# haidog-yaqub/EzAudio

Measured on NVIDIA H100. Metric: audio-seconds generated per wall-second (EzAudio-XL, 50-step DDIM, 10 s), higher is better.
Workload: dtype bf16

## Files before the change

### ezaudio_b200/csrc/gemm.cuh

```cuda
#pragma once
#include "common.cuh"

namespace ezb {

constexpr int GEMM_BM = 128;
constexpr int GEMM_BK = 64;
#ifdef EZB_GEMM_DEBUG
#define EZB_DBG(...) __VA_ARGS__
#else
#define EZB_DBG(...)
#endif
constexpr int GEMM_SMEM_BUDGET = 227 * 1024 - 2048;
constexpr int gemm_b_box(int bn) { return bn > 256 ? bn / 2 : bn; }

struct GemmShape {
  int M, N;
  int num_k_blocks;
  int num_m_tiles, num_n_tiles;
  int taps, center, dilation, cin_blocks, T, tiles_per_batch;
  int stride, pad;
  unsigned long long* dbg;
  const char* pf;
  unsigned int pf_bytes;
};
// ... 371 lines not shown
    float rstd = 1.f, nmr = 0.f;
    if (fold && lane < nvalid) fold_row_stats(ep.fin, row0 + lane, rstd, nmr);
    wait();
    const int f_begin = c_begin / 2, f_end = c_end / 2;
#pragma unroll 1
    for (int c = f_begin; c < f_end; c += 64) {
      if (n0 + c >= N) break;
      if (ep.split_stride > 0) {
        uint32_t h[32], g[32];
#pragma unroll 1
        for (int q4 = 0; q4 < 2; ++q4) {
          __syncwarp();
          acc_ld<32>(ar, c + q4 * 32, lane, h);
          acc_ld<32>(ar, HALF + c + q4 * 32, lane, g);
          if (lane < nvalid) {
            __nv_bfloat16* o = ep.out_bf16 + (size_t)(row0 + lane) * ep.ld16 + (n0 / 2 + c + q4 * 32);
#pragma unroll
            for (int j = 0; j < 32; j += 2) {
              const float o0 = (__uint_as_float(h[j]) + ep.bias[n0 + c + q4 * 32 + j]) * gelu_erf(__uint_as_float(g[j]) + ep.bias[n0 + HALF + c + q4 * 32 + j]);
              const float o1 = (__uint_as_float(h[j + 1]) + ep.bias[n0 + c + q4 * 32 + j + 1]) * gelu_erf(__uint_as_float(g[j + 1]) + ep.bias[n0 + HALF + c + q4 * 32 + j + 1]);
              store_bf16x2(o + j, ep.split_stride, o0, o1);
            }
          }
        }
        continue;
      }
      uint32_t pk[32];
#pragma unroll
      for (int q4 = 0; q4 < 2; ++q4) {
        uint32_t h[32], g[32];
        __syncwarp();
        acc_ld<32>(ar, c + q4 * 32, lane, h);
        acc_ld<32>(ar, HALF + c + q4 * 32, lane, g);
        if (fold) {
          const float* bh = ep.fin.v + n0 + c + q4 * 32;
          const float* bg = ep.fin.v + n0 + HALF + c + q4 * 32;
          const float* uh = ep.fin.u + n0 + c + q4 * 32;
          const float* ug = ep.fin.u + n0 + HALF + c + q4 * 32;
#pragma unroll
          for (int j = 0; j < 32; j += 2) {
            const float o0 = geglu_fast(fmaf(__uint_as_float(h[j]), rstd, fmaf(nmr, __ldg(uh + j), __ldg(bh + j))),
                                        fmaf(__uint_as_float(g[j]), rstd, fmaf(nmr, __ldg(ug + j), __ldg(bg + j))));
            const float o1 = geglu_fast(fmaf(__uint_as_float(h[j + 1]), rstd, fmaf(nmr, __ldg(uh + j + 1), __ldg(bh + j + 1))),
                                        fmaf(__uint_as_float(g[j + 1]), rstd, fmaf(nmr, __ldg(ug + j + 1), __ldg(bg + j + 1))));
            pk[q4 * 16 + j / 2] = pack_bf16(o0, o1);
          }
        } else {
        const float* bh = ep.bias + n0 + c + q4 * 32;
        const float* bg = ep.bias + n0 + HALF + c + q4 * 32;
#pragma unroll
        for (int j = 0; j < 32; j += 2) {
          const float o0 = geglu_fast(__uint_as_float(h[j]) + __ldg(bh + j), __uint_as_float(g[j]) + __ldg(bg + j));
          const float o1 = geglu_fast(__uint_as_float(h[j + 1]) + __ldg(bh + j + 1), __uint_as_float(g[j + 1]) + __ldg(bg + j + 1));
          pk[q4 * 16 + j / 2] = pack_bf16(o0, o1);
        }
        }
      }
      __syncwarp();
#pragma unroll
      for (int gq = 0; gq < 16; ++gq) stage_put<32>(st, lane, gq, __uint_as_float(pk[2 * gq]), __uint_as_float(pk[2 * gq + 1]));
      __syncwarp();
      const int hl = lane & 15, hw = lane >> 4;
      __nv_bfloat16* obase = ep.out_bf16 + (size_t)row0 * ep.ld16 + (n0 / 2 + c + 4 * hl);
#pragma unroll 4
      for (int rp = 0; rp < 16; ++rp) {
        const int rr = 2 * rp + hw;
        if (rr < nvalid) *reinterpret_cast<float2*>(obase + (size_t)rr * ep.ld16) = stage_get<32>(st, rr, hl);
      }
    }
  }
};

__device__ __forceinline__ void warpgroup_bar_sync(int wg) {
  if (wg == 0) named_bar_sync(2, 128);
  else named_bar_sync(3, 128);
}
struct EpiGegluFrag {
  using Params = EpiGegluParams;
  static constexpr bool FRAG = true;
  static constexpr int EPI_WARPS = 8;
  static constexpr bool WIDE_REGS = false;
  static constexpr int STAGE_FLOATS = 32 * 32;
  static constexpr int HALF = 128;
  static __device__ __forceinline__ void frag(const Params& ep, const CUtensorMap* out, float (&d)[128], uint8_t* tile, int m0, int n0, int wg, int lg,
                                              int lane) {
    const int q = lane & 3;
    const int r0 = 16 * lg + (lane >> 2);
    const float2* bh = reinterpret_cast<const float2*>(ep.bias + n0) + q;
    const float2* bg = reinterpret_cast<const float2*>(ep.bias + n0 + HALF) + q;
#pragma unroll
    for (int i = 0; i < 16; ++i) {
      const float2 b_h = __ldg(bh + 4 * i), b_g = __ldg(bg + 4 * i);
      const uint32_t lo = pack_bf16(geglu_fast(d[4 * i] + b_h.x, d[64 + 4 * i] + b_g.x), geglu_fast(d[4 * i + 1] + b_h.y, d[64 + 4 * i + 1] + b_g.y));
      const uint32_t hi = pack_bf16(geglu_fast(d[4 * i + 2] + b_h.x, d[64 + 4 * i + 2] + b_g.x), geglu_fast(d[4 * i + 3] + b_h.y, d[64 + 4 * i + 3] + b_g.y));
      uint8_t* p = tile + (i >> 3) * 8192 + r0 * 128 + (((i & 7) ^ (r0 & 7)) << 4) + 4 * q;
      *reinterpret_cast<uint32_t*>(p) = lo;
      *reinterpret_cast<uint32_t*>(p + 8 * 128) = hi;
    }
    fence_proxy_async_smem();
    warpgroup_bar_sync(wg);
    if ((threadIdx.x & 127) == 0) {
      tma_store_2d(out, tile, n0 / 2, m0 + 64 * wg);
      tma_store_2d(out, tile + 8192, n0 / 2 + 64, m0 + 64 * wg);
      bulk_commit_group();
    }
  }
};
template <class E>
constexpr auto epi_frag_impl(int) -> decltype(E::FRAG) { return E::FRAG; }
template <class E>
constexpr bool epi_frag_impl(long) { return false; }
template <class E>
constexpr bool epi_frag() { return epi_frag_impl<E>(0); }

__device__ __forceinline__ int swap_chunk_tokens(int c, int c_end, int t0, int N) {
  int n = c_end - c;
  if (N - t0 < n) n = N - t0;
  return n < 32 ? n : 32;
}
template <int BN>
struct EpiLinearT {
  using Params = EpiLinearParams;
  static constexpr int EPI_WARPS = 8;
  static constexpr bool WIDE_REGS = false;
  static constexpr int STAGE_FLOATS = 0;
  static __device__ __forceinline__ void load_resid(const Params& ep, float (&x)[32], int t0, int nt, int f, bool f_ok) {
#pragma unroll
    for (int j = 0; j < 32; ++j) x[j] = (f_ok && j < nt) ? ep.resid[(size_t)(t0 + j) * ep.ldr + f] : 0.f;
  }
  template <class Wait>
  static __device__ __forceinline__ void run(const Params& ep, float* st, const AccRows& ar, int row0, int nvalid, int n0, int N, int lane, int c_begin,
                                             int c_end, Wait wait) {
    const int f = row0 + lane;
    const bool f_ok = lane < nvalid;
    const float bias = (ep.bias != nullptr && f_ok) ? ep.bias[f] : 0.f;
    bool waited = false;
    float x[32];
    if (ep.resid != nullptr && n0 + c_begin < N) load_resid(ep, x, n0 + c_begin, swap_chunk_tokens(c_begin, c_end, n0 + c_begin, N), f, f_ok);
#pragma unroll 1
    for (int c = c_begin; c < c_end; c += 32) {
      const int t0 = n0 + c;
      if (t0 >= N) break;
      const int nt = swap_chunk_tokens(c, c_end, t0, N);
      float xn[32];
      const bool more = ep.resid != nullptr && c + 32 < c_end && t0 + 32 < N;
      if (more) load_resid(ep, xn, t0 + 32, swap_chunk_tokens(c + 32, c_end, t0 + 32, N), f, f_ok);
      float g0 = 1.f, g1 = 1.f;
      int btok = 0x7fffffff;
      if (ep.gate != nullptr && f_ok) {
        const int b0i = t0 / ep.rows_per_batch;
        btok = (b0i + 1) * ep.rows_per_batch;
        g0 = 1.0f - ep.gate[(size_t)b0i * ep.gate_bstride + f];
        if (btok < t0 + nt) g1 = 1.0f - ep.gate[(size_t)(b0i + 1) * ep.gate_bstride + f];
      }
      if (!waited) { wait(); waited = true; }
      uint32_t r[32];
      __syncwarp();
      acc_ld<32>(ar, c, lane, r);
      if (f_ok) {
        float* o = ep.out_f32 + (size_t)t0 * ep.ld32 + f;
#pragma unroll
        for (int j = 0; j < 32; ++j) {
          if (j >= nt) break;
          float v = __uint_as_float(r[j]) + bias;
          if (ep.resid != nullptr) v = fmaf((t0 + j >= btok) ? g1 : g0, v, x[j]);
          o[(size_t)j * ep.ld32] = v;
        }
      }
// ... 239 lines not shown
  constexpr uint16_t MC_MASK = static_cast<uint16_t>((1u << MC) - 1u);
  uint8_t* smem = smem_raw + ((1024u - (smem_u32(smem_raw) & 1023u)) & 1023u);
  uint8_t* sA = smem;
  uint8_t* sB = smem + STAGES * SM::A_BYTES;
  float* sAcc = reinterpret_cast<float*>(smem);
  float* sStage = reinterpret_cast<float*>(smem + SM::RING);
  uint64_t* full = reinterpret_cast<uint64_t*>(smem + SM::RING + SM::STAGE_BYTES);
  uint64_t* empty = full + STAGES;
  uint64_t* acc_free = empty + STAGES;

  const int warp = threadIdx.x >> 5;
  const int lane = threadIdx.x & 31;
  const int num_tiles = g.num_m_tiles * g.num_n_tiles;
  constexpr int PRODUCER = EPI_WARPS;

  if (warp == PRODUCER && lane == 0) {
    tma_prefetch_desc(&tmA);
    tma_prefetch_desc(&tmB);
    for (int i = 0; i < STAGES; ++i) {
      mbar_init(&full[i], 1);
      mbar_init(&empty[i], SM::MMA_WG * MC);
    }
    mbar_init(acc_free, EPI_WARPS * MC);
    fence_mbar_init();
  }
  __syncthreads();
  if (MC > 1) cluster_sync_all();
  pdl_launch();
  if (warp == PRODUCER && g.pf_bytes != 0) {
    if (elect_one()) prefetch_weights_l2(g.pf, g.pf_bytes, blockIdx.x, gridDim.x);
    __syncwarp();
  }
  pdl_wait();
  EZB_DBG(const bool dbg = g.dbg != nullptr && blockIdx.x == 0; const long long t_start = clock64(); long long w0 = 0, w1 = 0, w4 = 0;)

  if (warp >= PRODUCER) {
    if constexpr (SM::PRODUCER_WG) setmaxnreg_dec<SM::REGS_PRODUCER>();
    uint32_t stage = 0, phase = 0, af_phase = 0;
    bool first = true;
    for (int tile = warp == PRODUCER ? (int)blockIdx.x : num_tiles; tile < num_tiles; tile += gridDim.x) {
      const int mt = tile % g.num_m_tiles, nt = tile / g.num_m_tiles;
      const int n0 = nt * BN;
      if (!SM::FRAG && !first) { mbar_wait(acc_free, af_phase); af_phase ^= 1; }
      first = false;
      for (int kb0 = 0; kb0 < g.num_k_blocks; kb0 += KSUB) {
        EZB_DBG(const long long tq = clock64();)
        mbar_wait(&empty[stage], phase ^ 1);
        EZB_DBG(w0 += clock64() - tq;)
        const int nsub = g.num_k_blocks - kb0 < KSUB ? g.num_k_blocks - kb0 : KSUB;
        if (elect_one()) {
          mbar_expect_tx(&full[stage], nsub * (SM::A_SUB + SM::B_SUB));
          for (int sub = 0; sub < nsub; ++sub) {
          const int kb = kb0 + sub;
          uint8_t* dA = sA + stage * SM::A_BYTES + sub * SM::A_SUB;
          uint8_t* dB = sB + stage * SM::B_BYTES + sub * SM::B_SUB;
          if (g.taps == 0) {
            tma_load_2d(dA, &tmA, &full[stage], kb * KB_ELEMS, mt * GEMM_BM);
          } else {
            const int tap = kb / g.cin_blocks, cb = kb - tap * g.cin_blocks;
            const int bidx = mt / g.tiles_per_batch, t0 = (mt - bidx * g.tiles_per_batch) * GEMM_BM;
            if (g.stride > 1) {
              const int off = tap - g.pad;
              const int r = ((off % g.stride) + g.stride) % g.stride, dq = (off - r) / g.stride;
              tma_load_4d(dA, &tmA, &full[stage], cb * GEMM_BK, r, t0 + dq, bidx);
            } else {
              tma_load_3d(dA, &tmA, &full[stage], cb * GEMM_BK, t0 + (tap - g.center) * g.dilation, bidx);
            }
          }
          if (MC == 1) {
            constexpr int BOX = gemm_b_box(BN);
#pragma unroll
            for (int j = 0; j < BN / BOX; ++j) tma_load_2d(dB + j * BOX * 128, &tmB, &full[stage], kb * KB_ELEMS, n0 + j * BOX);
          } else {
            constexpr int SR = McSub<BN>::ROWS;
            for (int j = (int)cluster_ctarank(); j < BN / SR; j += MC)
              tma_load_2d_mc(dB + j * SR * 128, &tmB, &full[stage], kb * KB_ELEMS, n0 + j * SR, MC_MASK);
          }
          }
        }
        __syncwarp();
        if (++stage == STAGES) { stage = 0; phase ^= 1; }
      }
    }
    if constexpr (SM::PRODUCER_WG) setmaxnreg_inc<SM::REGS_LAUNCH>();
  } else {
    if constexpr (SM::PRODUCER_WG) setmaxnreg_inc<SM::REGS_CONSUMER>();
    const int wg = warp >> 2, lg = warp & 3;
    uint32_t stage = 0, phase = 0;
    if constexpr (SM::FRAG) {
      static_assert(!FP8 && !FIRST_PHASE && KSUB == 1, "FRAG: bf16 kernels of one phase (gemm_frag_kernel)");
      uint8_t* tile_buf = reinterpret_cast<uint8_t*>(sStage) + wg * (SM::STAGE_BYTES / 2);
      for (int tile = blockIdx.x; tile < num_tiles; tile += gridDim.x) {
        const int mt = tile % g.num_m_tiles, nt = tile / g.num_m_tiles;
        EZB_DBG(const long long tm = clock64();)
        float d[NSUB][SM::NH][SM::HN / 2];
        gemm_mainloop<BN, Epi, MC, KSUB>(d, wg * NSUB, sA, sB, full, empty, g.num_k_blocks, stage, phase);
        EZB_DBG(const long long ta = clock64(); w0 += ta - tm;)
        if ((threadIdx.x & 127) == 0) bulk_wait_group_read<0>();
        warpgroup_bar_sync(wg);
        EZB_DBG(const long long te = clock64(); w1 += te - ta;)
        Epi::frag(ep, tmC, d[0][0], tile_buf, mt * GEMM_BM, nt * BN, wg, lg, lane);
        EZB_DBG(w4 += clock64() - te;)
      }
      if ((threadIdx.x & 127) == 0) bulk_wait_group<0>();
    } else
    for (int tile = blockIdx.x; tile < num_tiles; tile += gridDim.x) {
      const int mt = tile % g.num_m_tiles, nt = tile / g.num_m_tiles;
      EZB_DBG(const long long tm = clock64();)
      gemm_mma_part<BN, Epi, MC, KSUB, FP8>(wg * NSUB, sA, sB, sAcc, full, empty, g.num_k_blocks, stage, phase, lg, lane, fs, mt * GEMM_BM, g.M, nt * BN);
      EZB_DBG(const long long ta = clock64(); w0 += ta - tm;)
      named_bar_sync(1, 32 * EPI_WARPS);
      EZB_DBG(const long long te = clock64(); w1 += te - ta;)
      int row0, nvalid;
      if (g.taps == 0) {
        row0 = mt * GEMM_BM + lg * 32;
        nvalid = g.M - row0;
      } else {
        const int bidx = mt / g.tiles_per_batch, t0 = (mt - bidx * g.tiles_per_batch) * GEMM_BM + lg * 32;
        row0 = bidx * g.T + t0;
        nvalid = g.T - t0;
      }
      constexpr int CW = BN / (EPI_WARPS / 4);
      const AccRows ar{sAcc + lg * 32 * SM::ACC_PITCH, SM::ACC_PITCH};
      Epi::run(ep, sStage + warp * Epi::STAGE_FLOATS, ar, row0, nvalid, nt * BN, g.N, lane, wg * CW, (wg + 1) * CW, []() {});
      EZB_DBG(w4 += clock64() - te;)
      fence_proxy_async_smem();
      __syncwarp();
      if (lane == 0) {
        if (MC == 1) mbar_arrive(acc_free);
        else for (int r = 0; r < MC; ++r) mbar_arrive_cluster(mapa_u32(smem_u32(acc_free), r));
      }
    }
    if constexpr (SM::PRODUCER_WG) setmaxnreg_dec<SM::REGS_LAUNCH>();
  }
  EZB_DBG(if (dbg && lane == 0) {
    if (warp == PRODUCER) atomicAdd(&g.dbg[2], (unsigned long long)w0);
    if (warp == 0) {
      atomicAdd(&g.dbg[0], (unsigned long long)w0); atomicAdd(&g.dbg[1], (unsigned long long)w1); atomicAdd(&g.dbg[4], (unsigned long long)w4);
      atomicAdd(&g.dbg[5], (unsigned long long)(clock64() - t_start));
    }
  })
  __syncthreads();
  if (MC > 1) cluster_sync_all();
  if (FIRST_PHASE) {
    if (warp == PRODUCER && lane == 0) {
      for (int i = 0; i < STAGES; ++i) { mbar_inval(&full[i]); mbar_inval(&empty[i]); }
      mbar_inval(acc_free);
    }
    __syncthreads();
  }
}
template <int BN, class Epi, int MC = 1, int KSUB = 1>
__global__ void __launch_bounds__((GemmCfg<BN, Epi, KSUB>::THREADS), 1)
gemm_wgmma_kernel(const __grid_constant__ CUtensorMap tmA, const __grid_constant__ CUtensorMap tmB, const GemmShape g,
                  const typename Epi::Params ep) {
  extern __shared__ uint8_t smem_dyn[];
  gemm_body<BN, Epi, MC, false, KSUB>(tmA, tmB, g, ep, smem_dyn);
}
template <int BN, class Epi>
__global__ void __launch_bounds__((GemmCfg<BN, Epi>::THREADS), 1)
gemm_frag_kernel(const __grid_constant__ CUtensorMap tmA, const __grid_constant__ CUtensorMap tmB, const __grid_constant__ CUtensorMap tmC,
                 const GemmShape g, const typename Epi::Params ep) {
  extern __shared__ uint8_t smem_dyn[];
  gemm_body<BN, Epi, 2>(tmA, tmB, g, ep, smem_dyn, Fp8Scales{}, &tmC);
}
template <int BN, class Epi>
__global__ void __launch_bounds__((GemmCfg<BN, Epi>::THREADS), 1)
gemm_fp8_kernel(const __grid_constant__ CUtensorMap tmA, const __grid_constant__ CUtensorMap tmB, const GemmShape g, const typename Epi::Params ep,
                const Fp8Scales fs) {
  extern __shared__ uint8_t smem_dyn[];
  gemm_body<BN, Epi, 2, false, 1, true>(tmA, tmB, g, ep, smem_dyn, fs);
}

}

namespace ezb {
struct EpiHeadsParams {
  int D, H, L;
  int kind[3];
  float nw[2][72];
  float nb[2][72];
  const float2* rope;
  int rope_ld;
  int rope_mufu;
  float inv_freq[36];
  int rope_kinds;
  __nv_bfloat16* out[3];
  int ld_qk, dvp, Lpad;
  int dbg;
  FoldIn fin;
};

template <int DH, int HPT = 2, bool DIRECT = false, bool FOLD = false, bool DBG = false>
struct EpiHeads {
  using Params = EpiHeadsParams;
  static constexpr int BN = HPT == 3 ? (DH == 72 ? 224 : 3 * DH) : 2 * DH;
  static constexpr int EPI_WARPS = 8;
  static constexpr bool WIDE_REGS = HPT == 3;
  static constexpr int STAGE_FLOATS = DIRECT ? 0 : EPI_STAGE_FLOATS;
  template <class Wait>
  static __device__ __forceinline__ void run(const Params& ep, float* st, const AccRows& ar, int row0, int nvalid, int n0, int N, int lane, int c_begin,
                                             int c_end, Wait wait) {
    const int row = row0 + lane;
    const bool row_ok = lane < nvalid;
    constexpr bool fold = FOLD;
    float f_rstd = 1.f, f_nmr = 0.f;
    if (fold && row_ok) fold_row_stats(ep.fin, row, f_rstd, f_nmr);
    wait();
    const int b = row_ok ? row / ep.L : 0, l = row_ok ? row - b * ep.L : 0;
#pragma unroll 1
    for (int hh = threadIdx.x >> 7; hh < HPT; hh += 2) {
      int sec, head;
      if (HPT == 3) {
        const int g = (n0 / BN) * 3 + hh;
        sec = g / ep.H;
        head = g - sec * ep.H;
      } else {
        const int n = n0 + hh * DH;
        if (n >= N) break;
        sec = n / ep.D;
        head = (n - sec * ep.D) / DH;
      }
      const int kind = ep.kind[sec];
      uint32_t r[DH];
      __syncwarp();
      acc_ld<64>(ar, hh * DH, lane, r);
      if constexpr (DH == 72) acc_ld<8>(ar, hh * DH + 64, lane, r + 64);
      float v[DH];
#pragma unroll
      for (int i = 0; i < DH; ++i) v[i] = __uint_as_float(r[i]);
      if (fold) {
        const float4* u4 = reinterpret_cast<const float4*>(ep.fin.u + n0 + hh * DH);
        const float4* v4 = reinterpret_cast<const float4*>(ep.fin.v + n0 + hh * DH);
#pragma unroll
        for (int i = 0; i < DH / 4; ++i) {
          const float4 uu = __ldg(u4 + i), vv = __ldg(v4 + i);
          v[4 * i] = fmaf(v[4 * i], f_rstd, fmaf(f_nmr, uu.x, vv.x));
          v[4 * i + 1] = fmaf(v[4 * i + 1], f_rstd, fmaf(f_nmr, uu.y, vv.y));
          v[4 * i + 2] = fmaf(v[4 * i + 2], f_rstd, fmaf(f_nmr, uu.z, vv.z));
          v[4 * i + 3] = fmaf(v[4 * i + 3], f_rstd, fmaf(f_nmr, uu.w, vv.w));
        }
      }
      const size_t bh = (size_t)b * ep.H + head;
      if (kind < 2) {
        float s1[4] = {0.f, 0.f, 0.f, 0.f}, s2[4] = {0.f, 0.f, 0.f, 0.f};
#pragma unroll
        for (int i = 0; i < DH; ++i) { s1[i & 3] += v[i]; s2[i & 3] = fmaf(v[i], v[i], s2[i & 3]); }
        const float mean = ((s1[0] + s1[1]) + (s1[2] + s1[3])) * (1.0f / DH);
        const float var = fmaxf(((s2[0] + s2[1]) + (s2[2] + s2[3])) * (1.0f / DH) - mean * mean, 0.f);
        const float rstd = rsqrtf(var + 1e-5f);
        const float nmr = -mean * rstd;
        if (DBG && (ep.dbg & 2)) {
        } else if (kind == 0) {
#pragma unroll
          for (int i = 0; i < DH; ++i) v[i] = fmaf(fmaf(v[i], rstd, nmr), ep.nw[0][i], ep.nb[0][i]);
        } else {
#pragma unroll
          for (int i = 0; i < DH; ++i) v[i] = fmaf(fmaf(v[i], rstd, nmr), ep.nw[1][i], ep.nb[1][i]);
        }
        if (ep.rope != nullptr && ((ep.rope_kinds >> kind) & 1) && !(DBG && (ep.dbg & 1))) {
          const float2* cs = ep.rope + (size_t)l * (DH / 2);
          const float lf = (float)l;
#pragma unroll
          for (int i = 0; i < DH / 2; ++i) {
            float2 c;
            if (ep.rope_mufu) __sincosf(lf * ep.inv_freq[i], &c.y, &c.x);
            else c = __ldg(cs + i);
            const float a = v[i], bq = v[i + DH / 2];
            v[i] = a * c.x - bq * c.y;
            v[i + DH / 2] = bq * c.x + a * c.y;
          }
        }
        if constexpr (DIRECT) {
          if (row_ok) {
            uint4* dst = reinterpret_cast<uint4*>(ep.out[kind] + (bh * ep.L + l) * (size_t)ep.ld_qk);
#pragma unroll
            for (int g = 0; g < DH / 8; ++g)
              dst[g] = make_uint4(pack_bf16(v[8 * g], v[8 * g + 1]), pack_bf16(v[8 * g + 2], v[8 * g + 3]), pack_bf16(v[8 * g + 4], v[8 * g + 5]),
                                  pack_bf16(v[8 * g + 6], v[8 * g + 7]));
          }
          continue;
        }
#pragma unroll
        for (int g = 0; g < DH / 4; ++g)
          stage_put(st, lane, g, __uint_as_float(pack_bf16(v[4 * g], v[4 * g + 1])), __uint_as_float(pack_bf16(v[4 * g + 2], v[4 * g + 3])));
        __syncwarp();
        if (lane < DH / 4 && !(DBG && (ep.dbg & 8))) {
          const int rb0 = row0 / ep.L, rl0 = row0 - rb0 * ep.L;
          __nv_bfloat16* base = ep.out[kind] + 4 * lane;
          const size_t head_rows = (size_t)ep.L * ep.ld_qk;
          const int nv = nvalid < 32 ? nvalid : 32;
#pragma unroll 4
          for (int rr = 0; rr < nv; ++rr) {
            int rl = rl0 + rr, rb = rb0;
            while (rl >= ep.L) { rl -= ep.L; ++rb; }
            *reinterpret_cast<float2*>(base + ((size_t)rb * ep.H + head) * head_rows + (size_t)rl * ep.ld_qk) = stage_get(st, rr, lane);
          }
        }
      } else if (row_ok && !(DBG && (ep.dbg & 4))) {
        __nv_bfloat16* dst = ep.out[2] + bh * ep.dvp * ep.Lpad + l;
#pragma unroll
        for (int i = 0; i < DH; ++i) { *dst = __float2bfloat16_rn(v[i]); dst += ep.Lpad; }
        for (int i = DH; i < ep.dvp; ++i) { *dst = __float2bfloat16_rn(0.f); dst += ep.Lpad; }
      }
    }
  }
};

}

namespace ezb {
struct GridBarrier { unsigned int count; unsigned int gen; };
__device__ __forceinline__ void grid_barrier(GridBarrier* b) {
  __syncthreads();
  if (threadIdx.x == 0) {
    __threadfence();
    unsigned int gen;
    asm volatile("ld.acquire.gpu.global.u32 %0, [%1];" : "=r"(gen) : "l"(&b->gen) : "memory");
    if (atomicAdd(&b->count, 1u) == gridDim.x - 1) {
      b->count = 0;
      __threadfence();
      asm volatile("st.release.gpu.global.u32 [%0], %1;" ::"l"(&b->gen), "r"(gen + 1) : "memory");
    } else {
      unsigned int cur;
      do {
        asm volatile("ld.acquire.gpu.global.u32 %0, [%1];" : "=r"(cur) : "l"(&b->gen) : "memory");
      } while (cur == gen);
    }
  }
  __syncthreads();
  asm volatile("fence.proxy.async;" ::: "memory");
}
template <int BN1, class Epi1, class Epi2>
__global__ void __launch_bounds__((GemmCfg<BN1, Epi1>::THREADS), 1)
mlp_fused_kernel(const __grid_constant__ CUtensorMap tmA1, const __grid_constant__ CUtensorMap tmB1, const GemmShape g1, const typename Epi1::Params ep1,
                 const __grid_constant__ CUtensorMap tmA2, const __grid_constant__ CUtensorMap tmB2, const GemmShape g2, const typename Epi2::Params ep2,
                 GridBarrier* bar) {
  static_assert(GemmCfg<BN1, Epi1>::THREADS == GemmCfg<256, Epi2>::THREADS, "both phases use the same warp roles");
  extern __shared__ uint8_t smem_dyn[];
  gemm_body<BN1, Epi1, 2, true>(tmA1, tmB1, g1, ep1, smem_dyn);
  grid_barrier(bar);
  gemm_body<256, Epi2, 1>(tmA2, tmB2, g2, ep2, smem_dyn);
}

}
```

### ezaudio_b200/csrc/host.cuh

```cuda
#pragma once
#include <cuda.h>
#include <cuda_runtime.h>
#include <stdarg.h>
#include <stdio.h>
#include <stdlib.h>
#include <string.h>

#include <map>
#include <string>
#include <tuple>
#include <utility>
#include <vector>

#include "../../include/ezb200.h"
#include "gemm.cuh"

namespace ezb {


inline unsigned long long& launch_counter() {
  static unsigned long long n = 0;
  return n;
}
inline int& opt_pair_gemm() {
// ... 323 lines not shown
  EZB_TRY(dev.tmaps.get2d(A, (uint64_t)K, (uint64_t)M_tokens, (uint64_t)lda, gemm_b_box(BN), &tB));
  return launch_gemm_t<BN, Epi>(dev, st, tA, tB, g, ep);
}

inline int swapped_bn(const Device& dev, int M_tokens, int N_features) {
  const long long mt = (N_features + GEMM_BM - 1) / GEMM_BM;
  auto span = [&](long long bn) { return (mt * ((M_tokens + bn - 1) / bn) + dev.num_sms - 1) / dev.num_sms * bn; };
  return span(288) < span(256) ? 288 : 256;
}
template <template <int> class Epi>
int gemm_swapped(Device& dev, cudaStream_t st, const __nv_bfloat16* A, int lda, const __nv_bfloat16* W, int ldw, int M_tokens, int N_features, int K,
                 const typename Epi<256>::Params& ep) {
  if (swapped_bn(dev, M_tokens, N_features) == 288) return gemm_swapped_at<288, Epi<288>>(dev, st, A, lda, W, ldw, M_tokens, N_features, K, ep);
  return gemm_swapped_at<256, Epi<256>>(dev, st, A, lda, W, ldw, M_tokens, N_features, K, ep);
}

inline int& opt_swap_mc() {
  static int v = 0;
  return v;
}
template <template <int> class EpiT, int MC>
int gemm_swapped_mc(Device& dev, cudaStream_t st, const __nv_bfloat16* A, int lda, const __nv_bfloat16* W, int ldw, int M_tokens, int N_features, int K,
                    const typename EpiT<256>::Params& ep) {
  constexpr int BN = 256;
  using Epi = EpiT<BN>;
  const int mt = (N_features + GEMM_BM - 1) / GEMM_BM, nt = (M_tokens + BN - 1) / BN, tiles = mt * nt;
  auto kern = gemm_wgmma_kernel<BN, Epi, MC>;
  constexpr int smem = GemmCfg<BN, Epi>::BYTES;
  constexpr int GEMM_THREADS = GemmCfg<BN, Epi>::THREADS;
  static int max_clusters[16] = {};
  int& mc = max_clusters[dev.id & 15];
  if (mc == 0) {
    mc = -1;
    if (cudaFuncSetAttribute(kern, cudaFuncAttributeMaxDynamicSharedMemorySize, smem) == cudaSuccess) {
      cudaLaunchConfig_t cfg;
      memset(&cfg, 0, sizeof cfg);
      cfg.gridDim = dim3(MC * 64); cfg.blockDim = dim3(GEMM_THREADS); cfg.dynamicSmemBytes = smem;
      cudaLaunchAttribute at;
      at.id = cudaLaunchAttributeClusterDimension; at.val.clusterDim.x = MC; at.val.clusterDim.y = 1; at.val.clusterDim.z = 1;
      cfg.attrs = &at; cfg.numAttrs = 1;
      int n = 0;
      if (cudaOccupancyMaxActiveClusters(&n, kern, &cfg) == cudaSuccess && n > 0) mc = n;
    }
    (void)cudaGetLastError();
  }
  if (mc <= 0 || (mt % MC) || tiles > mc * MC || (K % 8) || (lda % 8) || (ldw % 8))
    return gemm_swapped<EpiT>(dev, st, A, lda, W, ldw, M_tokens, N_features, K, ep);
  GemmShape g;
  memset(&g, 0, sizeof g);
  g.M = N_features; g.N = M_tokens;
  g.num_m_tiles = mt; g.num_n_tiles = nt;
  g.num_k_blocks = (K + GEMM_BK - 1) / GEMM_BK;
  const CUtensorMap *tA, *tB;
  EZB_TRY(dev.tmaps.get2d(W, (uint64_t)K, (uint64_t)N_features, (uint64_t)ldw, GEMM_BM, &tA));
  EZB_TRY(dev.tmaps.get2d(A, (uint64_t)K, (uint64_t)M_tokens, (uint64_t)lda, 32, &tB));
  GemmProf& gp = gemm_prof();
  cudaEvent_t e0 = nullptr, e1 = nullptr;
  if (gp.on) {
    if (gp.used + 2 > gp.ev.size()) {
      for (int i = 0; i < 2; ++i) { cudaEvent_t e; EZB_CUDA(cudaEventCreate(&e)); gp.ev.push_back(e); }
    }
    e0 = gp.ev[gp.used]; e1 = gp.ev[gp.used + 1];
    gp.used += 2;
    gp.flops.push_back(2.0 * (double)g.M * (double)g.N * (double)g.num_k_blocks * GEMM_BK);
    EZB_CUDA(cudaEventRecord(e0, st));
  }
  EZB_TRY(launch_k(kern, dim3(tiles), dim3(GEMM_THREADS), smem, st, MC, *tA, *tB, g, ep));
  if (gp.on) EZB_CUDA(cudaEventRecord(e1, st));
  return EZB_OK;
}

template <class Kern>
int resident_clusters2(Device& dev, Kern kern, int smem, int threads, int* n) {
  cudaLaunchConfig_t cfg;
  memset(&cfg, 0, sizeof cfg);
  cfg.gridDim = dim3(dev.num_sms & ~1); cfg.blockDim = dim3(threads); cfg.dynamicSmemBytes = smem;
  cudaLaunchAttribute at;
  at.id = cudaLaunchAttributeClusterDimension; at.val.clusterDim.x = 2; at.val.clusterDim.y = 1; at.val.clusterDim.z = 1;
  cfg.attrs = &at; cfg.numAttrs = 1;
  EZB_CUDA(cudaOccupancyMaxActiveClusters(n, kern, &cfg));
  if (*n <= 0) return fail(EZB_ERR_CUDA, "no 2-CTA cluster of this GEMM fits on the device");
  return EZB_OK;
}
template <int BN, class Epi, int KSUB = 1>
int gemm2(Device& dev, cudaStream_t st, const __nv_bfloat16* A, int lda, const __nv_bfloat16* W, int ldw, int M, int N, int K,
          const typename Epi::Params& ep) {
  if (M <= 0 || N <= 0 || K <= 0) return fail(EZB_ERR_SHAPE, "gemm2: empty problem %d %d %d", M, N, K);
  if ((K % 8) || (lda % 8) || (ldw % 8) || (N % 8)) return fail(EZB_ERR_SHAPE, "gemm2: K/ld/N must be multiples of 8 (M%d N%d K%d)", M, N, K);
  GemmShape g;
  memset(&g, 0, sizeof g);
  g.M = M; g.N = N;
  g.num_n_tiles = (N + BN - 1) / BN;
  g.dbg = gemm_dbg_buf();
  g.num_m_tiles = ((M + GEMM_BM - 1) / GEMM_BM + 1) & ~1;
  g.num_k_blocks = (K + GEMM_BK - 1) / GEMM_BK;
  dev.next_weights(W, (size_t)N * ldw * 2, &g.pf, &g.pf_bytes);
  const CUtensorMap *tA, *tB;
  EZB_TRY(dev.tmaps.get2d(A, (uint64_t)K, (uint64_t)M, (uint64_t)lda, GEMM_BM, &tA));
  EZB_TRY(dev.tmaps.get2d(W, (uint64_t)K, (uint64_t)N, (uint64_t)ldw, McSub<BN>::ROWS, &tB));
  constexpr bool FRAG = GemmCfg<BN, Epi, KSUB>::FRAG;
  const CUtensorMap* tC = nullptr;
  if constexpr (FRAG) {
    if (ep.split_stride != 0 || ep.fin.u != nullptr || N % BN)
      return fail(EZB_ERR_ARG, "gemm2: the fragment GEGLU epilogue writes plain bf16 of whole %d-column tiles (N %d)", BN, N);
    EZB_TRY(dev.tmaps.get2d(ep.out_bf16, (uint64_t)N / 2, (uint64_t)M, (uint64_t)ep.ld16, 64, &tC));
  }
  auto kern = [] {
    if constexpr (FRAG) return gemm_frag_kernel<BN, Epi>;
    else return gemm_wgmma_kernel<BN, Epi, 2, KSUB>;
  }();
  constexpr int smem = GemmCfg<BN, Epi, KSUB>::BYTES;
  constexpr int GEMM_THREADS = GemmCfg<BN, Epi, KSUB>::THREADS;
  static int clusters[16] = {};
  if (!clusters[dev.id & 15]) {
    EZB_CUDA(cudaFuncSetAttribute(kern, cudaFuncAttributeMaxDynamicSharedMemorySize, smem));
    EZB_TRY(resident_clusters2(dev, kern, smem, GEMM_THREADS, &clusters[dev.id & 15]));
  }
  const int tiles = g.num_m_tiles * g.num_n_tiles, max_ctas = 2 * clusters[dev.id & 15];
  const int ctas = tiles < max_ctas ? tiles : max_ctas;
  GemmProf& gp = gemm_prof();
  cudaEvent_t e0 = nullptr, e1 = nullptr;
  if (gp.on) {
    if (gp.used + 2 > gp.ev.size()) {
      for (int i = 0; i < 2; ++i) { cudaEvent_t e; EZB_CUDA(cudaEventCreate(&e)); gp.ev.push_back(e); }
    }
    e0 = gp.ev[gp.used]; e1 = gp.ev[gp.used + 1];
    gp.used += 2;
    gp.flops.push_back(2.0 * (double)M * (double)N * (double)g.num_k_blocks * GEMM_BK);
    EZB_CUDA(cudaEventRecord(e0, st));
  }
  if constexpr (FRAG) EZB_TRY(launch_k(kern, dim3(ctas), dim3(GEMM_THREADS), smem, st, 2, *tA, *tB, *tC, g, ep));
  else EZB_TRY(launch_k(kern, dim3(ctas), dim3(GEMM_THREADS), smem, st, 2, *tA, *tB, g, ep));
  if (gp.on) EZB_CUDA(cudaEventRecord(e1, st));
  return EZB_OK;
}

inline int gemm2_geglu(Device& dev, cudaStream_t st, const __nv_bfloat16* A, int lda, const __nv_bfloat16* W, int ldw, int M, int N, int K,
                       const EpiGegluParams& p) {
  const bool tma_out = (reinterpret_cast<uintptr_t>(p.out_bf16) & 15) == 0 && p.ld16 % 8 == 0;
  if (p.split_stride == 0 && N % 256 == 0 && tma_out) return gemm2<256, EpiGegluFrag>(dev, st, A, lda, W, ldw, M, N, K, p);
  return gemm2<256, EpiGeglu<256>>(dev, st, A, lda, W, ldw, M, N, K, p);
}

template <int BN, class Epi>
int gemm2_fp8(Device& dev, cudaStream_t st, const uint8_t* A, const float* sa, const uint8_t* W, const float* sw, int M, int N, int K,
              const typename Epi::Params& ep) {
  if (M <= 0 || N <= 0 || K <= 0) return fail(EZB_ERR_SHAPE, "gemm2_fp8: empty problem %d %d %d", M, N, K);
  if ((K % 16) || (N % BN)) return fail(EZB_ERR_SHAPE, "gemm2_fp8: K must be a multiple of 16 and N of %d (M%d N%d K%d)", BN, M, N, K);
  GemmShape g;
  memset(&g, 0, sizeof g);
  g.M = M; g.N = N;
  g.num_n_tiles = N / BN;
  g.num_m_tiles = ((M + GEMM_BM - 1) / GEMM_BM + 1) & ~1;
  g.num_k_blocks = (K + 2 * GEMM_BK - 1) / (2 * GEMM_BK);
  dev.next_weights(W, (size_t)N * K, &g.pf, &g.pf_bytes);
  const CUtensorMap *tA, *tB;
  EZB_TRY(dev.tmaps.get2d_u8(A, (uint64_t)K, (uint64_t)M, (uint64_t)K, GEMM_BM, &tA));
  EZB_TRY(dev.tmaps.get2d_u8(W, (uint64_t)K, (uint64_t)N, (uint64_t)K, McSub<BN>::ROWS, &tB));
  auto kern = gemm_fp8_kernel<BN, Epi>;
  constexpr int smem = GemmCfg<BN, Epi>::BYTES;
  constexpr int GEMM_THREADS = GemmCfg<BN, Epi>::THREADS;
  static int clusters[16] = {};
  if (!clusters[dev.id & 15]) {
    EZB_CUDA(cudaFuncSetAttribute(kern, cudaFuncAttributeMaxDynamicSharedMemorySize, smem));
    EZB_TRY(resident_clusters2(dev, kern, smem, GEMM_THREADS, &clusters[dev.id & 15]));
  }
  const int tiles = g.num_m_tiles * g.num_n_tiles, max_ctas = 2 * clusters[dev.id & 15];
  const int ctas = tiles < max_ctas ? tiles : max_ctas;
  GemmProf& gp = gemm_prof();
  cudaEvent_t e0 = nullptr, e1 = nullptr;
  if (gp.on) {
    if (gp.used + 2 > gp.ev.size()) {
      for (int i = 0; i < 2; ++i) { cudaEvent_t e; EZB_CUDA(cudaEventCreate(&e)); gp.ev.push_back(e); }
    }
    e0 = gp.ev[gp.used]; e1 = gp.ev[gp.used + 1];
    gp.used += 2;
    gp.flops.push_back(2.0 * (double)M * (double)N * (double)K);
    EZB_CUDA(cudaEventRecord(e0, st));
  }
  const Fp8Scales fs{sa, sw};
  EZB_TRY(launch_k(kern, dim3(ctas), dim3(GEMM_THREADS), smem, st, 2, *tA, *tB, g, ep, fs));
  if (gp.on) EZB_CUDA(cudaEventRecord(e1, st));
  return EZB_OK;
}

inline int& opt_mlp_fused() {
  static int v = [] { const char* e = getenv("EZB_MLP_FUSED"); return e ? atoi(e) : 0; }();
  return v;
}
template <class Epi1, class Epi2>
int mlp_fused(Device& dev, cudaStream_t st, const __nv_bfloat16* A1, const __nv_bfloat16* W1, int M, int N1, int K1, const typename Epi1::Params& ep1,
              const __nv_bfloat16* mid, const __nv_bfloat16* W2, int N2, int K2, const typename Epi2::Params& ep2, GridBarrier* bar) {
  constexpr int BN1 = 256, BN2 = 256;
  if ((K1 % 8) || (K2 % 8) || (N1 % 8)) return fail(EZB_ERR_SHAPE, "mlp_fused: K / N must be multiples of 8");
  GemmShape g1, g2;
  memset(&g1, 0, sizeof g1);
  memset(&g2, 0, sizeof g2);
  g1.M = M; g1.N = N1;
  g1.num_n_tiles = (N1 + BN1 - 1) / BN1; g1.num_m_tiles = ((M + GEMM_BM - 1) / GEMM_BM + 1) & ~1; g1.num_k_blocks = (K1 + GEMM_BK - 1) / GEMM_BK;
  g2.M = N2; g2.N = M;
  g2.num_m_tiles = (N2 + GEMM_BM - 1) / GEMM_BM; g2.num_n_tiles = (M + BN2 - 1) / BN2; g2.num_k_blocks = (K2 + GEMM_BK - 1) / GEMM_BK;
  const CUtensorMap *tA1, *tB1, *tA2, *tB2;
  EZB_TRY(dev.tmaps.get2d(A1, (uint64_t)K1, (uint64_t)M, (uint64_t)K1, GEMM_BM, &tA1));
  EZB_TRY(dev.tmaps.get2d(W1, (uint64_t)K1, (uint64_t)N1, (uint64_t)K1, McSub<BN1>::ROWS, &tB1));
  EZB_TRY(dev.tmaps.get2d(W2, (uint64_t)K2, (uint64_t)N2, (uint64_t)K2, GEMM_BM, &tA2));
  EZB_TRY(dev.tmaps.get2d(mid, (uint64_t)K2, (uint64_t)M, (uint64_t)K2, BN2, &tB2));
  auto kern = mlp_fused_kernel<BN1, Epi1, Epi2>;
  constexpr int s1 = GemmCfg<BN1, Epi1>::BYTES, s2 = GemmCfg<BN2, Epi2>::BYTES, smem = s1 > s2 ? s1 : s2;
  constexpr int THREADS = GemmCfg<BN1, Epi1>::THREADS;
  static int clusters[16] = {};
  if (!clusters[dev.id & 15]) {
    EZB_CUDA(cudaFuncSetAttribute(kern, cudaFuncAttributeMaxDynamicSharedMemorySize, smem));
    EZB_TRY(resident_clusters2(dev, kern, smem, THREADS, &clusters[dev.id & 15]));
  }
  const int grid = 2 * clusters[dev.id & 15];
  return launch_k(kern, dim3(grid), dim3(THREADS), smem, st, 2, *tA1, *tB1, g1, ep1, *tA2, *tB2, g2, ep2, bar);
}

template <int BN, class Epi>
int gemm(Device& dev, cudaStream_t st, const __nv_bfloat16* A, int lda, const __nv_bfloat16* W, int ldw, int M, int N, int K,
         const typename Epi::Params& ep, const ConvAddr* conv = nullptr) {
  if (M <= 0 || N <= 0 || K <= 0) return fail(EZB_ERR_SHAPE, "gemm: empty problem %d %d %d", M, N, K);
  if ((K % 8) || (lda % 8) || (ldw % 8) || (N % 8)) return fail(EZB_ERR_SHAPE, "gemm: K/ld/N must be multiples of 8 (M%d N%d K%d)", M, N, K);
  GemmShape g;
  memset(&g, 0, sizeof g);
  g.M = M;
  g.N = N;
  g.num_n_tiles = (N + BN - 1) / BN;
  dev.next_weights(W, (size_t)N * ldw * 2, &g.pf, &g.pf_bytes);
  const CUtensorMap *tA, *tB;
  if (conv && conv->taps > 0) {
    g.taps = conv->taps;
    g.center = conv->center;
    g.dilation = conv->dilation;
    g.cin_blocks = conv->cin_pad / GEMM_BK;
    g.T = conv->T;
    g.tiles_per_batch = (conv->T + GEMM_BM - 1) / GEMM_BM;
    g.num_m_tiles = g.tiles_per_batch * conv->B;
    g.num_k_blocks = conv->taps * g.cin_blocks;
    g.stride = conv->stride;
    g.pad = conv->pad;
    if (conv->stride > 1) {
      TmapCache::Key k(A, (uint64_t)K, (uint64_t)conv->T, (uint64_t)conv->B, (uint64_t)lda * 1000003ull + conv->stride, GEMM_BM, 4);
      auto it = dev.tmaps.maps.find(k);
      if (it == dev.tmaps.maps.end()) {
        CUtensorMap m;
        EZB_TRY(make_tmap4_strided(&m, A, (uint64_t)K, (uint64_t)conv->stride, (uint64_t)conv->T, (uint64_t)conv->B, (uint64_t)lda));
        it = dev.tmaps.maps.emplace(k, m).first;
      }
      tA = &it->second;
    } else
    EZB_TRY(dev.tmaps.get3d(A, (uint64_t)K, (uint64_t)conv->T, (uint64_t)conv->B, (uint64_t)lda, (uint64_t)lda * conv->T, GEMM_BM, &tA));
    EZB_TRY(dev.tmaps.get2d(W, (uint64_t)conv->taps * conv->cin_pad, (uint64_t)N, (uint64_t)ldw, BN, &tB));
  } else {
    g.num_m_tiles = (M + GEMM_BM - 1) / GEMM_BM;
    g.num_k_blocks = (K + GEMM_BK - 1) / GEMM_BK;
    EZB_TRY(dev.tmaps.get2d(A, (uint64_t)K, (uint64_t)M, (uint64_t)lda, GEMM_BM, &tA));
    EZB_TRY(dev.tmaps.get2d(W, (uint64_t)K, (uint64_t)N, (uint64_t)ldw, BN, &tB));
  }
  return launch_gemm_t<BN, Epi>(dev, st, tA, tB, g, ep);
}

enum HeadsVariant {
  HEADS_PACKED3 = 0,
  HEADS_PACKED3_DIRECT = 1,
  HEADS_PACKED3_KSUB2 = 2,
  HEADS_PAIR = 3,
  HEADS_PAIR_DIRECT = 4,
  HEADS_SINGLE = 5,
};
inline int heads_gemm(Device& dev, cudaStream_t st, const __nv_bfloat16* A, const __nv_bfloat16* W, int M, int N, int dh, int variant,
                      const EpiHeadsParams& e) {
  const int D = e.D, H = e.H;
  const bool fo = e.fin.u != nullptr;
  const bool packed = variant == HEADS_PACKED3 || variant == HEADS_PACKED3_DIRECT || variant == HEADS_PACKED3_KSUB2;
  const bool direct = variant == HEADS_PACKED3_DIRECT || variant == HEADS_PAIR_DIRECT;
  if (dh != 72 && dh != 64) return fail(EZB_ERR_UNSUPPORTED, "heads_gemm: head dimension %d", dh);
  if (packed && N != 3 * D) return fail(EZB_ERR_SHAPE, "heads_gemm: the packed-3 layout holds q, k and v (N %d, D %d)", N, D);
#define EZB_HEADS(BN_, DH_, HPT_, N_)                                                                                                          \
  (fo ? (direct ? gemm2<BN_, EpiHeads<DH_, HPT_, true, true>>(dev, st, A, D, W, D, M, N_, D, e) : gemm2<BN_, EpiHeads<DH_, HPT_, false, true>>(dev, st, A, D, W, D, M, N_, D, e)) \
      : (direct ? gemm2<BN_, EpiHeads<DH_, HPT_, true, false>>(dev, st, A, D, W, D, M, N_, D, e) : gemm2<BN_, EpiHeads<DH_, HPT_, false, false>>(dev, st, A, D, W, D, M, N_, D, e)))
  if (e.dbg) {
    if (variant != HEADS_PACKED3 || dh != 72 || fo) return fail(EZB_ERR_UNSUPPORTED, "heads_gemm: the profiling epilogue is packed-3, dh 72, unfolded");
    return gemm2<224, EpiHeads<72, 3, false, false, true>>(dev, st, A, D, W, D, M, H * 224, D, e);
  }
  switch (variant) {
    case HEADS_PACKED3_KSUB2:
      if (dh != 72 || fo) return fail(EZB_ERR_UNSUPPORTED, "heads_gemm: 128-deep slots exist for dh 72 without fold only");
      return gemm2<224, EpiHeads<72, 3, true, false>, 2>(dev, st, A, D, W, D, M, H * 224, D, e);
    case HEADS_PACKED3:
    case HEADS_PACKED3_DIRECT:
      if (dh == 72) return EZB_HEADS(224, 72, 3, H * 224);
      return EZB_HEADS(192, 64, 3, H * 192);
    case HEADS_PAIR:
    case HEADS_PAIR_DIRECT:
      if (dh == 72) return EZB_HEADS(144, 72, 2, N);
      return EZB_HEADS(128, 64, 2, N);
    case HEADS_SINGLE:
      if (fo) return fail(EZB_ERR_UNSUPPORTED, "heads_gemm: the single-CTA heads kernel has no fold");
      if (dh == 72) return gemm<144, EpiHeads<72>>(dev, st, A, D, W, D, M, N, D, e);
      return gemm<128, EpiHeads<64>>(dev, st, A, D, W, D, M, N, D, e);
  }
#undef EZB_HEADS
  return fail(EZB_ERR_ARG, "heads_gemm: variant %d", variant);
}
inline int heads_gemm_fp8(Device& dev, cudaStream_t st, const uint8_t* A, const float* sa, const uint8_t* W, const float* sw, int M, int dh,
                          const EpiHeadsParams& e) {
  if (e.fin.u != nullptr || e.dbg) return fail(EZB_ERR_UNSUPPORTED, "heads_gemm_fp8: no fold or profiling epilogue");
  if (dh == 72) return gemm2_fp8<224, EpiHeads<72, 3>>(dev, st, A, sa, W, sw, M, e.H * 224, e.D, e);
  if (dh == 64) return gemm2_fp8<192, EpiHeads<64, 3>>(dev, st, A, sa, W, sw, M, e.H * 192, e.D, e);
  return fail(EZB_ERR_UNSUPPORTED, "heads_gemm_fp8: head dimension %d", dh);
}

}
```

Baseline: 49.22.

## Add register-fragment epilogue for QKV heads GEMM with per-head LN and RoPE

Adds an EpiHeadsFrag epilogue that keeps the wgmma accumulators in registers and stages one head slice at a time through a small padded shared-memory buffer. Each thread then applies LayerNorm and RoPE to its row and stores it directly. This replaces the generic accumulator-staging path for the packed-3 and pair heads variants when there is no fold and outputs are 16-byte aligned. It also factors the per-head math into shared helpers and moves the producer's register re-raise to after the final syncthreads. The new path adds extra warpgroup barriers per head and zero-initializes the accumulators, which may raise register pressure.

```diff
diff --git a/ezaudio_b200/csrc/gemm.cuh b/ezaudio_b200/csrc/gemm.cuh
--- a/ezaudio_b200/csrc/gemm.cuh
+++ b/ezaudio_b200/csrc/gemm.cuh
@@ -477,8 +477,8 @@
   static constexpr bool WIDE_REGS = false;
   static constexpr int STAGE_FLOATS = 32 * 32;
   static constexpr int HALF = 128;
-  static __device__ __forceinline__ void frag(const Params& ep, const CUtensorMap* out, float (&d)[128], uint8_t* tile, int m0, int n0, int wg, int lg,
-                                              int lane) {
+  static __device__ __forceinline__ void frag(const Params& ep, const CUtensorMap* out, float (&d)[128], uint8_t* tile, int m0, int n0, const GemmShape&,
+                                              int wg, int lg, int lane) {
     const int q = lane & 3;
     const int r0 = 16 * lg + (lane >> 2);
     const float2* bh = reinterpret_cast<const float2*>(ep.bias + n0) + q;
@@ -884,7 +884,6 @@
         if (++stage == STAGES) { stage = 0; phase ^= 1; }
       }
     }
-    if constexpr (SM::PRODUCER_WG) setmaxnreg_inc<SM::REGS_LAUNCH>();
   } else {
     if constexpr (SM::PRODUCER_WG) setmaxnreg_inc<SM::REGS_CONSUMER>();
     const int wg = warp >> 2, lg = warp & 3;
@@ -895,13 +894,13 @@
       for (int tile = blockIdx.x; tile < num_tiles; tile += gridDim.x) {
         const int mt = tile % g.num_m_tiles, nt = tile / g.num_m_tiles;
         EZB_DBG(const long long tm = clock64();)
-        float d[NSUB][SM::NH][SM::HN / 2];
+        float d[NSUB][SM::NH][SM::HN / 2] = {};
         gemm_mainloop<BN, Epi, MC, KSUB>(d, wg * NSUB, sA, sB, full, empty, g.num_k_blocks, stage, phase);
         EZB_DBG(const long long ta = clock64(); w0 += ta - tm;)
         if ((threadIdx.x & 127) == 0) bulk_wait_group_read<0>();
         warpgroup_bar_sync(wg);
         EZB_DBG(const long long te = clock64(); w1 += te - ta;)
-        Epi::frag(ep, tmC, d[0][0], tile_buf, mt * GEMM_BM, nt * BN, wg, lg, lane);
+        Epi::frag(ep, tmC, d[0][0], tile_buf, mt * GEMM_BM, nt * BN, g, wg, lg, lane);
         EZB_DBG(w4 += clock64() - te;)
       }
       if ((threadIdx.x & 127) == 0) bulk_wait_group<0>();
@@ -943,6 +942,7 @@
     }
   })
   __syncthreads();
+  if constexpr (SM::PRODUCER_WG) if (warp >= PRODUCER) setmaxnreg_inc<SM::REGS_LAUNCH>();
   if (MC > 1) cluster_sync_all();
   if (FIRST_PHASE) {
     if (warp == PRODUCER && lane == 0) {
@@ -993,10 +993,72 @@
   FoldIn fin;
 };
 
+constexpr int heads_bn(int dh, int hpt) { return hpt == 3 ? (dh == 72 ? 224 : 3 * dh) : 2 * dh; }
+template <int DH, int HPT>
+__device__ __forceinline__ bool head_of_tile(const EpiHeadsParams& ep, int n0, int hh, int N, int& sec, int& head) {
+  if (HPT == 3) {
+    const int g = (n0 / heads_bn(DH, HPT)) * 3 + hh;
+    sec = g / ep.H;
+    head = g - sec * ep.H;
+    return true;
+  }
+  const int n = n0 + hh * DH;
+  if (n >= N) return false;
+  sec = n / ep.D;
+  head = (n - sec * ep.D) / DH;
+  return true;
+}
+template <int DH, bool DBG>
+__device__ __forceinline__ void head_ln_rope(const EpiHeadsParams& ep, float (&v)[DH], int kind, int l) {
+  float s1[4] = {0.f, 0.f, 0.f, 0.f}, s2[4] = {0.f, 0.f, 0.f, 0.f};
+#pragma unroll
+  for (int i = 0; i < DH; ++i) { s1[i & 3] += v[i]; s2[i & 3] = fmaf(v[i], v[i], s2[i & 3]); }
+  const float mean = ((s1[0] + s1[1]) + (s1[2] + s1[3])) * (1.0f / DH);
+  const float var = fmaxf(((s2[0] + s2[1]) + (s2[2] + s2[3])) * (1.0f / DH) - mean * mean, 0.f);
+  const float rstd = rsqrtf(var + 1e-5f);
+  const float nmr = -mean * rstd;
+  if (DBG && (ep.dbg & 2)) {
+  } else if (kind == 0) {
+#pragma unroll
+    for (int i = 0; i < DH; ++i) v[i] = fmaf(fmaf(v[i], rstd, nmr), ep.nw[0][i], ep.nb[0][i]);
+  } else {
+#pragma unroll
+    for (int i = 0; i < DH; ++i) v[i] = fmaf(fmaf(v[i], rstd, nmr), ep.nw[1][i], ep.nb[1][i]);
+  }
+  if (ep.rope != nullptr && ((ep.rope_kinds >> kind) & 1) && !(DBG && (ep.dbg & 1))) {
+    const float2* cs = ep.rope + (size_t)l * (DH / 2);
+    const float lf = (float)l;
+#pragma unroll
+    for (int i = 0; i < DH / 2; ++i) {
+      float2 c;
+      if (ep.rope_mufu) __sincosf(lf * ep.inv_freq[i], &c.y, &c.x);
+      else c = __ldg(cs + i);
+      const float a = v[i], bq = v[i + DH / 2];
+      v[i] = a * c.x - bq * c.y;
+      v[i + DH / 2] = bq * c.x + a * c.y;
+    }
+  }
+}
+template <int DH>
+__device__ __forceinline__ void head_store_row(const EpiHeadsParams& ep, const float (&v)[DH], int kind, size_t bh, int l) {
+  uint4* dst = reinterpret_cast<uint4*>(ep.out[kind] + (bh * ep.L + l) * (size_t)ep.ld_qk);
+#pragma unroll
+  for (int g = 0; g < DH / 8; ++g)
+    dst[g] = make_uint4(pack_bf16(v[8 * g], v[8 * g + 1]), pack_bf16(v[8 * g + 2], v[8 * g + 3]), pack_bf16(v[8 * g + 4], v[8 * g + 5]),
+                        pack_bf16(v[8 * g + 6], v[8 * g + 7]));
+}
+template <int DH>
+__device__ __forceinline__ void head_store_vt(const EpiHeadsParams& ep, const float (&v)[DH], size_t bh, int l) {
+  __nv_bfloat16* dst = ep.out[2] + bh * ep.dvp * ep.Lpad + l;
+#pragma unroll
+  for (int i = 0; i < DH; ++i) { *dst = __float2bfloat16_rn(v[i]); dst += ep.Lpad; }
+  for (int i = DH; i < ep.dvp; ++i) { *dst = __float2bfloat16_rn(0.f); dst += ep.Lpad; }
+}
+
 template <int DH, int HPT = 2, bool DIRECT = false, bool FOLD = false, bool DBG = false>
 struct EpiHeads {
   using Params = EpiHeadsParams;
-  static constexpr int BN = HPT == 3 ? (DH == 72 ? 224 : 3 * DH) : 2 * DH;
+  static constexpr int BN = heads_bn(DH, HPT);
   static constexpr int EPI_WARPS = 8;
   static constexpr bool WIDE_REGS = HPT == 3;
   static constexpr int STAGE_FLOATS = DIRECT ? 0 : EPI_STAGE_FLOATS;
@@ -1013,16 +1075,7 @@
 #pragma unroll 1
     for (int hh = threadIdx.x >> 7; hh < HPT; hh += 2) {
       int sec, head;
-      if (HPT == 3) {
-        const int g = (n0 / BN) * 3 + hh;
-        sec = g / ep.H;
-        head = g - sec * ep.H;
-      } else {
-        const int n = n0 + hh * DH;
-        if (n >= N) break;
-        sec = n / ep.D;
-        head = (n - sec * ep.D) / DH;
-      }
+      if (!head_of_tile<DH, HPT>(ep, n0, hh, N, sec, head)) break;
       const int kind = ep.kind[sec];
       uint32_t r[DH];
       __syncwarp();
@@ -1045,42 +1098,9 @@
       }
       const size_t bh = (size_t)b * ep.H + head;
       if (kind < 2) {
-        float s1[4] = {0.f, 0.f, 0.f, 0.f}, s2[4] = {0.f, 0.f, 0.f, 0.f};
-#pragma unroll
-        for (int i = 0; i < DH; ++i) { s1[i & 3] += v[i]; s2[i & 3] = fmaf(v[i], v[i], s2[i & 3]); }
-        const float mean = ((s1[0] + s1[1]) + (s1[2] + s1[3])) * (1.0f / DH);
-        const float var = fmaxf(((s2[0] + s2[1]) + (s2[2] + s2[3])) * (1.0f / DH) - mean * mean, 0.f);
-        const float rstd = rsqrtf(var + 1e-5f);
-        const float nmr = -mean * rstd;
-        if (DBG && (ep.dbg & 2)) {
-        } else if (kind == 0) {
-#pragma unroll
-          for (int i = 0; i < DH; ++i) v[i] = fmaf(fmaf(v[i], rstd, nmr), ep.nw[0][i], ep.nb[0][i]);
-        } else {
-#pragma unroll
-          for (int i = 0; i < DH; ++i) v[i] = fmaf(fmaf(v[i], rstd, nmr), ep.nw[1][i], ep.nb[1][i]);
-        }
-        if (ep.rope != nullptr && ((ep.rope_kinds >> kind) & 1) && !(DBG && (ep.dbg & 1))) {
-          const float2* cs = ep.rope + (size_t)l * (DH / 2);
-          const float lf = (float)l;
-#pragma unroll
-          for (int i = 0; i < DH / 2; ++i) {
-            float2 c;
-            if (ep.rope_mufu) __sincosf(lf * ep.inv_freq[i], &c.y, &c.x);
-            else c = __ldg(cs + i);
-            const float a = v[i], bq = v[i + DH / 2];
-            v[i] = a * c.x - bq * c.y;
-            v[i + DH / 2] = bq * c.x + a * c.y;
-          }
-        }
+        head_ln_rope<DH, DBG>(ep, v, kind, l);
         if constexpr (DIRECT) {
-          if (row_ok) {
-            uint4* dst = reinterpret_cast<uint4*>(ep.out[kind] + (bh * ep.L + l) * (size_t)ep.ld_qk);
-#pragma unroll
-            for (int g = 0; g < DH / 8; ++g)
-              dst[g] = make_uint4(pack_bf16(v[8 * g], v[8 * g + 1]), pack_bf16(v[8 * g + 2], v[8 * g + 3]), pack_bf16(v[8 * g + 4], v[8 * g + 5]),
-                                  pack_bf16(v[8 * g + 6], v[8 * g + 7]));
-          }
+          if (row_ok) head_store_row<DH>(ep, v, kind, bh, l);
           continue;
         }
 #pragma unroll
@@ -1100,10 +1120,64 @@
           }
         }
       } else if (row_ok && !(DBG && (ep.dbg & 4))) {
-        __nv_bfloat16* dst = ep.out[2] + bh * ep.dvp * ep.Lpad + l;
-#pragma unroll
-        for (int i = 0; i < DH; ++i) { *dst = __float2bfloat16_rn(v[i]); dst += ep.Lpad; }
-        for (int i = DH; i < ep.dvp; ++i) { *dst = __float2bfloat16_rn(0.f); dst += ep.Lpad; }
+        head_store_vt<DH>(ep, v, bh, l);
+      }
+    }
+  }
+};
+
+template <int DH, int HPT>
+struct EpiHeadsFrag {
+  using Params = EpiHeadsParams;
+  static constexpr bool FRAG = true;
+  static constexpr int BN = heads_bn(DH, HPT);
+  static constexpr int EPI_WARPS = 8;
+  static constexpr bool WIDE_REGS = true;
+  static constexpr int PITCH = DH + 4;
+  static constexpr int STAGE_FLOATS = 64 * PITCH / 4;
+  static_assert(DH % 8 == 0, "head slices start on a fragment register quad");
+  static __device__ __forceinline__ void frag(const Params& ep, const CUtensorMap*, float (&d)[BN / 2], uint8_t* tile, int m0, int n0, const GemmShape& g,
+                                              int wg, int lg, int lane) {
+    float* buf = reinterpret_cast<float*>(tile);
+    const int t = threadIdx.x & 127, half = t >> 6;
+    const int row = m0 + 64 * wg + (t & 63);
+    const bool row_ok = row < g.M;
+    const int b = row_ok ? row / ep.L : 0, l = row_ok ? row - b * ep.L : 0;
+    float* w0 = buf + (16 * lg + (lane >> 2)) * PITCH + 2 * (lane & 3);
+    const float4* rd = reinterpret_cast<const float4*>(buf + (t & 63) * PITCH);
+#pragma unroll
+    for (int p = 0; p < HPT; p += 2) {
+      float v[DH];
+#pragma unroll
+      for (int s = 0; s < 2; ++s) {
+        const int hh = p + s;
+        if (hh >= HPT) break;
+        if (hh > 0) warpgroup_bar_sync(wg);
+#pragma unroll
+        for (int i = 0; i < DH / 8; ++i) {
+          const int j = 4 * (hh * DH / 8 + i);
+          *reinterpret_cast<float2*>(w0 + 8 * i) = make_float2(d[j], d[j + 1]);
+          *reinterpret_cast<float2*>(w0 + 8 * PITCH + 8 * i) = make_float2(d[j + 2], d[j + 3]);
+        }
+        warpgroup_bar_sync(wg);
+        if (half == s) {
+#pragma unroll
+          for (int i = 0; i < DH / 4; ++i) {
+            const float4 x = rd[i];
+            v[4 * i] = x.x; v[4 * i + 1] = x.y; v[4 * i + 2] = x.z; v[4 * i + 3] = x.w;
+          }
+        }
+      }
+      const int hh = p + half;
+      int sec, head;
+      if (hh >= HPT || !head_of_tile<DH, HPT>(ep, n0, hh, g.N, sec, head)) continue;
+      const int kind = ep.kind[sec];
+      const size_t bh = (size_t)b * ep.H + head;
+      if (kind < 2) {
+        head_ln_rope<DH, false>(ep, v, kind, l);
+        if (row_ok) head_store_row<DH>(ep, v, kind, bh, l);
+      } else if (row_ok) {
+        head_store_vt<DH>(ep, v, bh, l);
       }
     }
   }
diff --git a/ezaudio_b200/csrc/host.cuh b/ezaudio_b200/csrc/host.cuh
--- a/ezaudio_b200/csrc/host.cuh
+++ b/ezaudio_b200/csrc/host.cuh
@@ -429,6 +429,17 @@
   if (*n <= 0) return fail(EZB_ERR_CUDA, "no 2-CTA cluster of this GEMM fits on the device");
   return EZB_OK;
 }
+inline int frag_out_map(Device& dev, const EpiGegluParams& ep, int M, int N, int BN, const CUtensorMap** tC) {
+  if (ep.split_stride != 0 || ep.fin.u != nullptr || N % BN)
+    return fail(EZB_ERR_ARG, "gemm2: the fragment GEGLU epilogue writes plain bf16 of whole %d-column tiles (N %d)", BN, N);
+  return dev.tmaps.get2d(ep.out_bf16, (uint64_t)N / 2, (uint64_t)M, (uint64_t)ep.ld16, 64, tC);
+}
+inline int frag_out_map(Device&, const EpiHeadsParams& ep, int, int N, int BN, const CUtensorMap** tC) {
+  *tC = nullptr;
+  if (ep.fin.u != nullptr || ep.dbg || N % BN)
+    return fail(EZB_ERR_ARG, "gemm2: the fragment heads epilogue has no fold or profiling variant and takes whole %d-column tiles (N %d)", BN, N);
+  return EZB_OK;
+}
 template <int BN, class Epi, int KSUB = 1>
 int gemm2(Device& dev, cudaStream_t st, const __nv_bfloat16* A, int lda, const __nv_bfloat16* W, int ldw, int M, int N, int K,
           const typename Epi::Params& ep) {
@@ -447,11 +458,7 @@
   EZB_TRY(dev.tmaps.get2d(W, (uint64_t)K, (uint64_t)N, (uint64_t)ldw, McSub<BN>::ROWS, &tB));
   constexpr bool FRAG = GemmCfg<BN, Epi, KSUB>::FRAG;
   const CUtensorMap* tC = nullptr;
-  if constexpr (FRAG) {
-    if (ep.split_stride != 0 || ep.fin.u != nullptr || N % BN)
-      return fail(EZB_ERR_ARG, "gemm2: the fragment GEGLU epilogue writes plain bf16 of whole %d-column tiles (N %d)", BN, N);
-    EZB_TRY(dev.tmaps.get2d(ep.out_bf16, (uint64_t)N / 2, (uint64_t)M, (uint64_t)ep.ld16, 64, &tC));
-  }
+  if constexpr (FRAG) EZB_TRY(frag_out_map(dev, ep, M, N, BN, &tC));
   auto kern = [] {
     if constexpr (FRAG) return gemm_frag_kernel<BN, Epi>;
     else return gemm_wgmma_kernel<BN, Epi, 2, KSUB>;
@@ -476,7 +483,7 @@
     gp.flops.push_back(2.0 * (double)M * (double)N * (double)g.num_k_blocks * GEMM_BK);
     EZB_CUDA(cudaEventRecord(e0, st));
   }
-  if constexpr (FRAG) EZB_TRY(launch_k(kern, dim3(ctas), dim3(GEMM_THREADS), smem, st, 2, *tA, *tB, *tC, g, ep));
+  if constexpr (FRAG) EZB_TRY(launch_k(kern, dim3(ctas), dim3(GEMM_THREADS), smem, st, 2, *tA, *tB, *(tC ? tC : tA), g, ep));
   else EZB_TRY(launch_k(kern, dim3(ctas), dim3(GEMM_THREADS), smem, st, 2, *tA, *tB, g, ep));
   if (gp.on) EZB_CUDA(cudaEventRecord(e1, st));
   return EZB_OK;
@@ -631,6 +638,15 @@
     if (variant != HEADS_PACKED3 || dh != 72 || fo) return fail(EZB_ERR_UNSUPPORTED, "heads_gemm: the profiling epilogue is packed-3, dh 72, unfolded");
     return gemm2<224, EpiHeads<72, 3, false, false, true>>(dev, st, A, D, W, D, M, H * 224, D, e);
   }
+  const bool rows16 = (reinterpret_cast<uintptr_t>(e.out[0]) & 15) == 0 && (reinterpret_cast<uintptr_t>(e.out[1]) & 15) == 0 && e.ld_qk % 8 == 0;
+  if (!fo && rows16 && variant == HEADS_PACKED3) {
+    if (dh == 72) return gemm2<224, EpiHeadsFrag<72, 3>>(dev, st, A, D, W, D, M, H * 224, D, e);
+    return gemm2<192, EpiHeadsFrag<64, 3>>(dev, st, A, D, W, D, M, H * 192, D, e);
+  }
+  if (!fo && rows16 && variant == HEADS_PAIR && N % (2 * dh) == 0) {
+    if (dh == 72) return gemm2<144, EpiHeadsFrag<72, 2>>(dev, st, A, D, W, D, M, N, D, e);
+    return gemm2<128, EpiHeadsFrag<64, 2>>(dev, st, A, D, W, D, M, N, D, e);
+  }
   switch (variant) {
     case HEADS_PACKED3_KSUB2:
       if (dh != 72 || fo) return fail(EZB_ERR_UNSUPPORTED, "heads_gemm: 128-deep slots exist for dh 72 without fold only");
```

New measurement: 51.38, median of 6. 1.04x the previous value.
